# mlrun/mlrun

Measured on NVIDIA H100. Metric: events/sec, higher is better.
Workload: dtype f32 in / f64 accumulate

## Files before the change

### mlrun_b200/csrc/b2s_rowthread.cuh

```cuda
#pragma once
#include <cuda.h>
#include <type_traits>

#include "b2s_device.cuh"
#include "b2s_hash.cuh"

namespace b2s {

constexpr int kRTMaxCatCols = 16;
constexpr int kRTCatsInline = 4;
constexpr int kRTMaxCats = 256;

template <int NCH, int NS>
struct RTParams {
  const char* rows;
  int64_t row_stride;
  int64_t n_rows;
  float* out;
  int32_t* status;
  int32_t n_in, out_cols, n_models, vote_kind, out_is_int, fast_epilogue, tile_rows, pitch, stages, vec_ok;
  int32_t n_cat_cols, n_cat;
  int32_t one_sync;
  int32_t use_bulk;
  float* peers[8];
  int64_t peer_off;
  int32_t n_peers;
  MergeSig sig;
  const double* wcat;
  const double* vote_w_g;
  const ModelDesc* models;
  const int32_t* classes;
  double w[NCH * 4][NS];
  float fill[NCH * 4];
  float lim[NCH * 4];
  double bias[NS];
  double vote_w[NS];
  int32_t cat_col[kRTMaxCatCols];
  int32_t cat_off[kRTMaxCatCols];
  int32_t cat_sw[kRTMaxCatCols];
  int32_t cat_base[kRTMaxCatCols];
  int32_t cat_cnt[kRTMaxCatCols];
  float cat_fill[kRTMaxCatCols];
  float cat_inl[kRTMaxCatCols][kRTCatsInline];
  int32_t cat_first[kRTMaxCatCols];
  int32_t cat_dense[kRTMaxCatCols];
  float cat_val[kRTMaxCats];
  struct CatFast {
    int32_t off_b;
    int32_t sw_b;
    int32_t first;
    int32_t cnt;
    int32_t woff_b;
    float fill;
    int32_t pad[2];
  };
  CatFast catf[kRTMaxCatCols];
  int32_t cats_fast;
  int32_t zero_woff_b;
  int32_t dead_tail;
  int32_t pad_fast;
  const long long* g_keys;
  const TableSlot* g_slots;
  uint64_t g_mask;
  const float* g_values;
  long long g_missing_row;
};

struct RowPadded {
  const float* xr;
  __device__ __forceinline__ float4 chunk(int ch) const { return *reinterpret_cast<const float4*>(xr + ch * 4); }
  __device__ __forceinline__ float at2(int off, int) const { return xr[off]; }
  __device__ __forceinline__ float at_b(int off_b, int) const { return *reinterpret_cast<const float*>(reinterpret_cast<const char*>(xr) + off_b); }
};
struct RowSwizzled {
  const float* box0;
  int box_words;
  int r7s;
  __device__ __forceinline__ float4 chunk(int ch) const {
    return *reinterpret_cast<const float4*>(box0 + (ch >> 3) * box_words + (((ch & 7) << 2) ^ r7s));
  }
  __device__ __forceinline__ float at2(int off, int sw) const { return box0[off + (sw ^ r7s)]; }
  __device__ __forceinline__ float at_b(int off_b, int sw_b) const {
    return *reinterpret_cast<const float*>(reinterpret_cast<const char*>(box0) + off_b + (sw_b ^ (r7s << 2)));
  }
};

template <int NCH, int NS, int CH0, int CH1, typename Row>
__device__ __forceinline__ void rt_slice(const RTParams<NCH, NS>& p, const Row (&xr)[1], double (&acc)[1][NS]) {
  constexpr int RPT = 1;
  constexpr int BATCH = 4;
#pragma unroll
  for (int b = CH0; b < CH1; b += BATCH) {
    double xd[RPT][BATCH * 4];
#pragma unroll
    for (int cb = 0; cb < BATCH; ++cb) {
      const int ch = b + cb;
      if (ch < CH1) {
#pragma unroll
        for (int i = 0; i < RPT; ++i) {
          const float4 v = xr[i].chunk(ch);
          const float xs[4] = {v.x, v.y, v.z, v.w};
#pragma unroll
          for (int u = 0; u < 4; ++u) {
            const int c = ch * 4 + u;
            float x = xs[u];
            x = !(fabsf(x) <= p.lim[c]) ? p.fill[c] : x;
            xd[i][cb * 4 + u] = (double)x;
          }
        }
      }
    }
#pragma unroll
    for (int cb = 0; cb < BATCH; ++cb) {
      const int ch = b + cb;
      if (ch < CH1) {
#pragma unroll
        for (int u = 0; u < 4; ++u) {
          const int c = ch * 4 + u;
#pragma unroll
          for (int k = 0; k < NS; ++k)
#pragma unroll
            for (int i = 0; i < RPT; ++i) acc[i][k] = fma(p.w[c][k], xd[i][cb * 4 + u], acc[i][k]);
        }
      }
    }
  }
}

template <int NCH, int NS>
__device__ __noinline__ int rt_cat_search(const RTParams<NCH, NS>& p, int cc, float x) {
  const int b0 = p.cat_base[cc], cnt = p.cat_cnt[cc];
  int j = p.n_cat;
  if (cnt <= kRTCatsInline) {
#pragma unroll
    for (int qq = kRTCatsInline - 1; qq >= 0; --qq) j = (x == p.cat_inl[cc][qq]) ? b0 + qq : j;
  } else {
    for (int qq = cnt - 1; qq >= 0; --qq) j = (x == p.cat_val[b0 + qq]) ? b0 + qq : j;
  }
  return j;
}

template <int NCH, int NS, int Q0, int TPR, typename Row>
__device__ __forceinline__ void rt_cats(const RTParams<NCH, NS>& p, const Row (&xr)[1], const double* __restrict__ s_wcat,
                                        double (&acc)[1][NS]) {
  constexpr int RPT = 1;
  constexpr int ITERS = (kRTMaxCatCols - Q0 + TPR - 1) / TPR;
  if (p.cats_fast) {
    const char* wb = reinterpret_cast<const char*>(s_wcat);
#pragma unroll
    for (int it = 0; it < ITERS; ++it) {
      const int cc = Q0 + it * TPR;
      if (cc >= p.n_cat_cols) break;
      const typename RTParams<NCH, NS>::CatFast cf = p.catf[cc];
#pragma unroll
      for (int i = 0; i < RPT; ++i) {
        float x = xr[i].at_b(cf.off_b, cf.sw_b);
        x = (x != x) ? cf.fill : x;
        const int v = __float2int_rz(x);
        const unsigned jj = (unsigned)(v - cf.first);
        const bool miss = ((float)v != x) | (jj >= (unsigned)cf.cnt);
        const int a = miss ? p.zero_woff_b : cf.woff_b + (int)jj * (NS * 8);
        if constexpr (NS % 2 == 0) {
#pragma unroll
          for (int k = 0; k < NS; k += 2) {
            const double2 w2 = *reinterpret_cast<const double2*>(wb + a + k * 8);
            acc[i][k] += w2.x;
            acc[i][k + 1] += w2.y;
          }
        } else {
          const double* wc = reinterpret_cast<const double*>(wb + a);
#pragma unroll
          for (int k = 0; k < NS; ++k) acc[i][k] += wc[k];
        }
      }
    }
    return;
  }
#pragma unroll
  for (int it = 0; it < ITERS; ++it) {
    const int cc = Q0 + it * TPR;
    if (cc >= p.n_cat_cols) break;
#pragma unroll
    for (int i = 0; i < RPT; ++i) {
      float x = xr[i].at2(p.cat_off[cc], p.cat_sw[cc]);
      x = (x != x) ? p.cat_fill[cc] : x;
      int j;
      if (p.cat_dense[cc]) {
        const int v = __float2int_rz(x);
        const unsigned jj = (unsigned)(v - p.cat_first[cc]);
        j = ((float)v == x && jj < (unsigned)p.cat_cnt[cc]) ? p.cat_base[cc] + (int)jj : p.n_cat;
      } else {
        j = rt_cat_search(p, cc, x);
      }
      const double* wc = s_wcat + (size_t)j * NS;
#pragma unroll
      for (int k = 0; k < NS; ++k) acc[i][k] += wc[k];
    }
  }
}

template <int NCH, int NS, int TPR, int LIVE, typename Row>
__device__ __forceinline__ void rt_row_slices(const RTParams<NCH, NS>& p, int q, const Row (&xr)[1], const double* __restrict__ s_wcat,
                                              double (&acc)[1][NS]) {
  static_assert(LIVE % TPR == 0, "live chunks must split evenly over the row's threads");
  constexpr int CPT = LIVE / TPR;
  if (TPR == 1 || q == 0) {
    rt_slice<NCH, NS, 0, CPT>(p, xr, acc);
    rt_cats<NCH, NS, 0, TPR>(p, xr, s_wcat, acc);
  } else if (q == 1) {
    rt_slice<NCH, NS, (TPR > 1 ? CPT : 0), (TPR > 1 ? 2 * CPT : 0)>(p, xr, acc);
    rt_cats<NCH, NS, (TPR > 1 ? 1 : 0), TPR>(p, xr, s_wcat, acc);
  } else if (q == 2) {
    rt_slice<NCH, NS, (TPR > 2 ? 2 * CPT : 0), (TPR > 2 ? 3 * CPT : 0)>(p, xr, acc);
    rt_cats<NCH, NS, (TPR > 2 ? 2 : 0), TPR>(p, xr, s_wcat, acc);
  } else {
    rt_slice<NCH, NS, (TPR > 3 ? 3 * CPT : 0), (TPR > 3 ? 4 * CPT : 0)>(p, xr, acc);
    rt_cats<NCH, NS, (TPR > 3 ? 3 : 0), TPR>(p, xr, s_wcat, acc);
  }
}

__device__ __forceinline__ void mbar_init(uint64_t* bar, int count) {
  asm volatile("mbarrier.init.shared::cta.b64 [%0], %1;" ::"r"((uint32_t)__cvta_generic_to_shared(bar)), "r"(count));
}
__device__ __forceinline__ void mbar_expect_tx(uint64_t* bar, uint32_t bytes) {
  asm volatile("mbarrier.arrive.expect_tx.shared::cta.b64 _, [%0], %1;" ::"r"((uint32_t)__cvta_generic_to_shared(bar)), "r"(bytes)
               : "memory");
}
__device__ __forceinline__ void mbar_wait(uint64_t* bar, uint32_t parity) {
  const uint32_t a = (uint32_t)__cvta_generic_to_shared(bar);
  asm volatile(
      "{\n"
      ".reg .pred p;\n"
      "WAIT_%=:\n"
      "mbarrier.try_wait.parity.shared::cta.b64 p, [%0], %1;\n"
      "@p bra DONE_%=;\n"
      "bra WAIT_%=;\n"
      "DONE_%=:\n"
      "}\n" ::"r"(a), "r"(parity)
      : "memory");
}
__device__ __forceinline__ void bulk_load(void* smem_dst, const void* gsrc, uint32_t bytes, uint64_t* bar) {
  asm volatile("cp.async.bulk.shared::cluster.global.mbarrier::complete_tx::bytes [%0], [%1], %2, [%3];" ::"r"(
                   (uint32_t)__cvta_generic_to_shared(smem_dst)),
               "l"(gsrc), "r"(bytes), "r"((uint32_t)__cvta_generic_to_shared(bar))
               : "memory");
}

__device__ __forceinline__ void tensor_load_2d(void* smem_dst, const CUtensorMap* tmap, int x, int y, uint64_t* bar) {
  asm volatile(
      "cp.async.bulk.tensor.2d.shared::cluster.global.tile.mbarrier::complete_tx::bytes [%0], [%1, {%2, %3}], [%4];" ::"r"(
          (uint32_t)__cvta_generic_to_shared(smem_dst)),
      "l"(reinterpret_cast<uint64_t>(tmap)), "r"(x), "r"(y), "r"((uint32_t)__cvta_generic_to_shared(bar))
      : "memory");
}

template <int NCH, int NS>
__device__ __noinline__ void rt_generic_epilogue(const RTParams<NCH, NS>& p, const double* sl, int64_t row, uint32_t st) {
  double pred[kMaxModels];
  for (int m = 0; m < p.n_models; ++m) {
    const ModelDesc md = p.models[m];
    pred[m] = apply_link(md, sl + md.score_off, p.classes);
  }
  KParams kp;
  kp.out = p.out;
  kp.out_cols = p.out_cols;
  kp.n_models = p.n_models;
  kp.vote_kind = p.vote_kind;
  kp.out_is_int = p.out_is_int;
  kp.vote_w = p.vote_w_g;
  kp.status = p.status;
  kp.n_peers = p.n_peers;
  kp.peer_off = p.peer_off;
  for (int g = 0; g < p.n_peers; ++g) kp.peers[g] = p.peers[g];
  vote_and_store(kp, pred, row, st);
}

template <int NCH, int NS, int TPR, int LM>
__global__ void __launch_bounds__(128 * TPR, TPR >= 4 ? 2 : (TPR == 2 ? 3 : 4))
    rowthread_kernel(const __grid_constant__ RTParams<NCH, NS> p, const __grid_constant__ CUtensorMap tmap) {
  constexpr int RPT = 1;
  static_assert(NCH % TPR == 0, "chunks must split evenly over the row's threads");
  constexpr int CPT = NCH / TPR;
  extern __shared__ __align__(16) unsigned char smem[];
  uint64_t* s_bar = reinterpret_cast<uint64_t*>(smem);
  double* s_wcat = reinterpret_cast<double*>(smem + 64);
  const size_t wcat_bytes = 64 + (((size_t)(p.n_cat + 1) * NS * 8 + 15) / 16) * 16;
  const bool one_sync = (LM == 2) && TPR > 1 && p.one_sync;
  constexpr size_t part_words = (size_t)(TPR - 1) * 128 * NS;
  double* s_part = reinterpret_cast<double*>(smem + wcat_bytes);
  float* s_tiles = reinterpret_cast<float*>(smem + wcat_bytes + (one_sync ? 2 : 1) * part_words * 8);
  if (LM == 2) {
    const uint32_t a = (uint32_t)__cvta_generic_to_shared(s_tiles);
    s_tiles += ((1024u - (a & 1023u)) & 1023u) >> 2;
  }

  const int tid = threadIdx.x;
  const int TR = p.tile_rows;
  const int S = p.stages;
  const int tile_words = (LM == 2) ? TR * NCH * 4 : TR * p.pitch;
  const int64_t n_tiles = (p.n_rows + TR - 1) / TR;
  const int TRT = TR / RPT;
  const int q = tid / TRT;
  const int r = tid - q * TRT;

  const int cprv = p.vec_ok ? (p.n_in >> 2) : p.n_in;
  const int r0 = tid / cprv, c0 = tid - r0 * cprv;
  const int dr = (int)blockDim.x / cprv, dc = (int)blockDim.x - dr * cprv;
  auto issue = [&](float* tile, int64_t row0) {
    int64_t left = p.n_rows - row0;
    const int rows = left < TR ? (left < 0 ? 0 : (int)left) : TR;
    const char* base = p.rows + row0 * p.row_stride;
    int rr = r0, cc = c0;
    if (p.vec_ok) {
      while (rr < rows) {
        cp_async16(tile + rr * p.pitch + cc * 4, base + (int64_t)rr * p.row_stride + cc * 16);
        rr += dr;
        cc += dc;
        if (cc >= cprv) {
          cc -= cprv;
          ++rr;
        }
      }
    } else {
      while (rr < rows) {
        cp_async4(tile + rr * p.pitch + cc, base + (int64_t)rr * p.row_stride + cc * 4);
        rr += dr;
        cc += dc;
        if (cc >= cprv) {
          cc -= cprv;
          ++rr;
        }
      }
    }
  };

  constexpr bool bulk = LM != 0;
  const uint32_t row_bytes = (uint32_t)p.n_in * 4u;
  uint32_t unknown_bits = 0;
  long long gk_cur = 0, gk_nxt = 0;
  longlong2 g_slot = make_longlong2(0, -1);
  uint64_t g_hash = 0;
  int64_t g_tile_nxt = 0;
  auto g_key = [&](int64_t tile) -> long long {
    const int64_t row = tile * TR + tid;
    return row < p.n_rows ? __ldg(p.g_keys + row) : 0;
  };
  auto g_probe_start = [&](long long key) {
    g_hash = mix64((uint64_t)key) & p.g_mask;
    g_slot = __ldg(reinterpret_cast<const longlong2*>(p.g_slots) + g_hash);
  };
  auto g_probe_finish = [&](long long key) -> long long {
    uint64_t h = g_hash;
    longlong2 sl = g_slot;
    for (;;) {
      if (sl.y < 0) return -1;
      if (sl.x == key) return sl.y;
      h = (h + 1) & p.g_mask;
      sl = __ldg(reinterpret_cast<const longlong2*>(p.g_slots) + h);
    }
  };
  if (LM == 1 && p.g_keys && tid < TR) {
    gk_cur = g_key(blockIdx.x);
    gk_nxt = g_key((int64_t)blockIdx.x + gridDim.x);
    g_probe_start(gk_cur);
    g_tile_nxt = (int64_t)blockIdx.x + 2 * (int64_t)gridDim.x;
  }
  auto issue_bulk = [&](int st, int64_t row0) {
    int64_t left = p.n_rows - row0;
    const int rows = left < TR ? (left < 0 ? 0 : (int)left) : TR;
    if (LM == 2) {
      if (tid == 0) {
        if (rows > 0) {
          mbar_expect_tx(&s_bar[st], (uint32_t)(NCH / 8) * (uint32_t)TR * 128u);
#pragma unroll
          for (int b = 0; b < NCH / 8; ++b)
            tensor_load_2d(s_tiles + st * tile_words + b * TR * 32, &tmap, b * 32, (int)row0, &s_bar[st]);
        } else {
          mbar_expect_tx(&s_bar[st], 0);
        }
      }
    } else {
      if (tid == 0) mbar_expect_tx(&s_bar[st], (uint32_t)rows * row_bytes);
      if (p.g_keys) {
        if (tid < TR) {
          const long long hit = g_probe_finish(gk_cur);
          if (tid < rows) {
            unknown_bits = (unknown_bits & ~(1u << st)) | ((hit < 0 ? 1u : 0u) << st);
            bulk_load(s_tiles + st * tile_words + tid * p.pitch,
                      reinterpret_cast<const char*>(p.g_values + (hit < 0 ? p.g_missing_row : hit) * p.n_in), row_bytes, &s_bar[st]);
          }
          gk_cur = gk_nxt;
          g_probe_start(gk_cur);
          gk_nxt = g_key(g_tile_nxt);
          g_tile_nxt += gridDim.x;
        }
      } else if (tid < rows) {
        bulk_load(s_tiles + st * tile_words + tid * p.pitch, p.rows + (row0 + tid) * p.row_stride, row_bytes, &s_bar[st]);
      }
    }
  };
  if (bulk) {
    if (tid == 0) {
      for (int s = 0; s < S; ++s) mbar_init(&s_bar[s], 1);
      asm volatile("fence.mbarrier_init.release.cluster;" ::: "memory");
    }
    __syncthreads();
  }
  for (int s = 0; s < (one_sync ? S : S - 1); ++s) {
    const int64_t t = (int64_t)blockIdx.x + (int64_t)s * gridDim.x;
    if (bulk) {
      issue_bulk(s, t * TR);
    } else {
      if (t < n_tiles) issue(s_tiles + s * tile_words, t * TR);
      cp_async_commit();
    }
  }
  uint32_t phase_bits = 0;
  for (int i = tid; i < p.n_cat * NS; i += blockDim.x) s_wcat[i] = p.wcat[i];
  for (int i = tid; i < NS; i += blockDim.x) s_wcat[p.n_cat * NS + i] = 0.0;
  if (one_sync) __syncthreads();

  int stage = 0;
  uint32_t iter = 0;
  for (int64_t t = blockIdx.x; t < n_tiles; t += gridDim.x) {
    if (bulk) {
      mbar_wait(&s_bar[stage], (phase_bits >> stage) & 1u);
      phase_bits ^= (1u << stage);
    } else if (S == 2) cp_async_wait<0>();
    else if (S == 3) cp_async_wait<1>();
    else cp_async_wait<2>();
    if (!one_sync) {
      __syncthreads();
      const int64_t tn = t + (int64_t)(S - 1) * gridDim.x;
      int sn = stage + S - 1;
      if (sn >= S) sn -= S;
      if (bulk) {
        issue_bulk(sn, tn * TR);
      } else {
        if (tn < n_tiles) issue(s_tiles + sn * tile_words, tn * TR);
        cp_async_commit();
      }
    }
    const float* tile = s_tiles + stage * tile_words;
    const int64_t row0 = t * TR;
    const int live_rows = (int)(p.n_rows - row0 < (int64_t)TR ? p.n_rows - row0 : (int64_t)TR);
    const bool any_live = r < live_rows;
    using Row = typename std::conditional<LM == 2, RowSwizzled, RowPadded>::type;
    Row xr[RPT];
#pragma unroll
    for (int i = 0; i < RPT; ++i) {
      const int ri = r + i * TRT;
      if constexpr (LM == 2) {
        xr[i].box0 = tile + ri * 32;
        xr[i].box_words = TR * 32;
        xr[i].r7s = (r & 7) << 2;
      } else {
        xr[i].xr = tile + ri * p.pitch;
      }
    }
    double acc[RPT][NS];
#pragma unroll
    for (int i = 0; i < RPT; ++i)
#pragma unroll
      for (int k = 0; k < NS; ++k) acc[i][k] = 0.0;
    if (any_live) {
      if constexpr (LM == 2 && RPT == 1 && NCH >= 8 && (TPR == 1 || TPR == 2)) {
        if (p.dead_tail >= 4) rt_row_slices<NCH, NS, TPR, NCH - 4>(p, q, xr, s_wcat, acc);
        else if (p.dead_tail >= 2) rt_row_slices<NCH, NS, TPR, NCH - 2>(p, q, xr, s_wcat, acc);
        else rt_row_slices<NCH, NS, TPR, NCH>(p, q, xr, s_wcat, acc);
      } else {
        rt_row_slices<NCH, NS, TPR, NCH>(p, q, xr, s_wcat, acc);
      }
    }
    if (TPR > 1) {
      double* s_part_cur = s_part + (one_sync ? (size_t)(iter & 1) * part_words : 0);
      if (q > 0) {
#pragma unroll
        for (int i = 0; i < RPT; ++i) {
          double* part = s_part_cur + ((size_t)(q - 1) * 128 + r + i * TRT) * NS;
#pragma unroll
          for (int k = 0; k < NS; ++k) part[k] = acc[i][k];
        }
      }
      __syncthreads();
      if (one_sync) issue_bulk(stage, (t + (int64_t)S * gridDim.x) * TR);
      if (q == 0) {
#pragma unroll
        for (int i = 0; i < RPT; ++i)
#pragma unroll
          for (int qq = 1; qq < TPR; ++qq) {
            const double* o = s_part_cur + ((size_t)(qq - 1) * 128 + r + i * TRT) * NS;
#pragma unroll
            for (int k = 0; k < NS; ++k) acc[i][k] += o[k];
          }
      }
    }
#pragma unroll
    for (int i = 0; i < RPT; ++i) {
      const int64_t row = row0 + (r + i * TRT);
      if (q == 0 && r + i * TRT < live_rows) {
        uint32_t st = 0;
#pragma unroll
        for (int k = 0; k < NS; ++k) {
          acc[i][k] += p.bias[k];
          st |= (fabs(acc[i][k]) <= 1.7976931348623157e308) ? 0u : 1u;
        }
        if (LM == 1) st |= ((unknown_bits >> stage) & 1u) << 2;
        if (p.fast_epilogue) {
          if (p.vote_kind == 1) {
            double s = 0.0;
#pragma unroll
            for (int k = 0; k < NS; ++k) s = __dadd_rn(s, __dmul_rn(acc[i][k], p.vote_w[k]));
            store_word(p, row, 0, __float_as_uint((float)s));
          } else {
#pragma unroll
            for (int k = 0; k < NS; ++k)
              if (k < p.n_models) store_word(p, row, k, __float_as_uint((float)acc[i][k]));
          }
          if (p.status) p.status[row] = (int32_t)st;
        } else {
          double sl[NS];
#pragma unroll
          for (int k = 0; k < NS; ++k) sl[k] = acc[i][k];
          rt_generic_epilogue(p, sl, row, st);
        }
      }
    }
    ++stage;
    ++iter;
    if (stage == S) stage = 0;
  }
  cp_async_wait<0>();
  merge_signal(p.sig);
}

}
```

### mlrun_b200/csrc/b2s_runtime.cu

```cuda
#include <cuda_runtime.h>

#include <exception>

#include <algorithm>
#include <atomic>
#include <chrono>
#include <cmath>
#include <condition_variable>
#include <cstdarg>
#include <cstdio>
#include <cstdlib>
#include <cstring>
#include <deque>
#include <limits>
#include <map>
#include <memory>
#include <mutex>
#include <string>
#include <thread>
#include <vector>

#include "../../include/b200serve.h"
#include "b2s_internal.h"
#include "b2s_device.cuh"
// ... 113 lines not shown

struct b2s_plan_s {
  int32_t n_in = 0;
  bool finalized = false;
  std::vector<float> fill;
  std::vector<std::vector<MapEntry>> maps;
  std::vector<int32_t> out_src, out_kind;
  std::vector<float> out_arg;
  std::vector<HostModel> models;
  int vote_kind = B2S_VOTE_NONE;
  std::vector<double> vote_w;
  int mode = MODE_STORE;
  int NS = 1;
  int out_cols = 0;
  int out_is_int = 0;
  KParams kp{};
  char* d_blob = nullptr;
  size_t blob_bytes = 0;
  int grid = 0, block = 0;
  int kernels_per_batch = 1;
  bool rt_ok = false;
  int rt_cat_cols = 0;
  int rt_NCH = 0, rt_NS = 0, rt_grid = 0, rt_smem = 0, rt_pitch = 0;
  std::vector<char> rt_blob;
  std::vector<void*> peers;
  int64_t peer_off = 0;
  struct b2s_comm_s* comm = nullptr;
  bool t2_ok = false;
  int t2_NS = 1, t2_grid = 0, t2_block = 512, t2_smem = 0;
  T2Params t2{};
  char* d_t2_blob = nullptr;
  struct TreeScratch {
    double* pred = nullptr;
    int32_t* row_bad = nullptr;
    uint32_t* xt = nullptr;
    int64_t rows = 0;
  };
  std::map<cudaStream_t, TreeScratch> t2_scratch;
  std::mutex scratch_mu;
  bool dense_ok = false;
  DenseParams dense{};
  int dense_smem = 0, dense_grid = 0;
  std::atomic<int32_t> last_kernel{B2S_KERNEL_NONE};
  bool t3_ok = false, t3_miss = false, t3_cat = false;
  bool any_cat = false;
  int t3_D = 0, t3_grid = 0, t3_block = 0, t3_smem = 0, t3_cols = 0, t3_parts = 0;
  T3Params t3{};
  T3Prep t3_prep{};
  int t3_prep_smem = 0;
  char* d_t3_blob = nullptr;
  const int32_t* d_t3_col_score = nullptr;
  const int32_t* d_t3_col_order = nullptr;
  const int32_t* d_t3_model_cols = nullptr;
  char* h_stage_in = nullptr;
  char* h_stage_out = nullptr;
  char* d_stage_in = nullptr;
  char* d_stage_out = nullptr;
  int32_t* d_stage_status = nullptr;
  int64_t stage_rows = 0;
  cudaEvent_t ev[4] = {nullptr, nullptr, nullptr, nullptr};
  std::vector<cudaEvent_t> chunk_ev;
  std::mutex host_mu;
  std::vector<Slot> slots;
  int open_slot = -1;
  uint64_t next_batch = 1;
  std::map<uint64_t, int> batch_slot;
  std::deque<int> sealed;
  std::mutex mu;
  std::condition_variable cv_work, cv_done, cv_free;
  std::thread dispatcher;
  bool stop = false;
  bool dispatch_busy = false;
  cudaStream_t ring_stream = nullptr;
  int64_t ring_cap = 0;
  std::atomic<int> spinners{0};
  int ring_cfg_slots = 0;
  int64_t ring_cfg_max_batch = 0;
  int ring_cfg_wait_us = -1;
  int wait_us() const { return ring_cfg_wait_us >= 0 ? ring_cfg_wait_us : G.max_wait_us; }
};

int b2s_int_plan_shape(b2s_plan_s* p, int* n_in, int* out_cols) {
  if (!p || !p->finalized) return fail(B2S_ERR_STATE, "plan not finalized");
  *n_in = p->n_in;
  *out_cols = p->out_cols;
  return B2S_OK;
}

static size_t align_up(size_t x, size_t a) { return (x + a - 1) / a * a; }

struct BlobBuilder {
  std::vector<char> data;
  template <typename T>
  size_t add(const std::vector<T>& v) {
    size_t off = align_up(data.size(), 16);
    data.resize(off + std::max<size_t>(v.size() * sizeof(T), 16));
    if (!v.empty()) memcpy(data.data() + off, v.data(), v.size() * sizeof(T));
    return off;
  }
};

template <int MODE, int NS>
static cudaError_t launch_rows(const KParams& kp, int grid, int block, cudaStream_t st) {
  static std::atomic<bool> attr_set{false};
  if (!attr_set) {
    cudaError_t e = cudaFuncSetAttribute(rows_kernel<MODE, NS>, cudaFuncAttributeMaxDynamicSharedMemorySize,
                                         (int)G.prop.sharedMemPerBlockOptin);
    if (e != cudaSuccess) return e;
    attr_set = true;
  }
  rows_kernel<MODE, NS><<<grid, block, kp.sm_total, st>>>(kp);
  return cudaGetLastError();
}

static cudaError_t launch_plan(b2s_plan_s* p, const KParams& kp, int grid, int block, cudaStream_t st) {
  G.launches.fetch_add(1, std::memory_order_relaxed);
#define B2S_CASE(M, N) \
  if (p->mode == M && p->NS == N) return launch_rows<M, N>(kp, grid, block, st);
  B2S_CASE(MODE_LINEAR, 1) B2S_CASE(MODE_LINEAR, 2) B2S_CASE(MODE_LINEAR, 4) B2S_CASE(MODE_LINEAR, 8)
  B2S_CASE(MODE_LINEAR, 16) B2S_CASE(MODE_LINEAR, 32)
  B2S_CASE(MODE_TREES, 1) B2S_CASE(MODE_TREES, 4) B2S_CASE(MODE_TREES, 8) B2S_CASE(MODE_TREES, 16)
  B2S_CASE(MODE_TREES, 32) B2S_CASE(MODE_STORE, 1)
#undef B2S_CASE
  return cudaErrorInvalidValue;
}

typedef CUresult (*EncodeTiledFn)(CUtensorMap*, CUtensorMapDataType, cuuint32_t, void*, const cuuint64_t*, const cuuint64_t*,
                                  const cuuint32_t*, const cuuint32_t*, CUtensorMapInterleave, CUtensorMapSwizzle,
                                  CUtensorMapL2promotion, CUtensorMapFloatOOBfill);
static EncodeTiledFn tensor_map_encoder() {
  static EncodeTiledFn fn = [] {
    void* sym = nullptr;
    cudaDriverEntryPointQueryResult q;
    if (cudaGetDriverEntryPoint("cuTensorMapEncodeTiled", &sym, cudaEnableDefault, &q) != cudaSuccess || q != cudaDriverEntryPointSuccess) {
      cudaGetLastError();
      sym = nullptr;
    }
    return reinterpret_cast<EncodeTiledFn>(sym);
  }();
  return fn;
}
static bool encode_rows_map(CUtensorMap* map, const void* rows, int64_t n_rows, int64_t stride, int n_in, int tile_rows) {
  EncodeTiledFn enc = tensor_map_encoder();
  if (!enc) return false;
  cuuint64_t gdim[2] = {(cuuint64_t)n_in, (cuuint64_t)n_rows};
  cuuint64_t gstride[1] = {(cuuint64_t)stride};
  cuuint32_t box[2] = {32u, (cuuint32_t)tile_rows};
  cuuint32_t estr[2] = {1u, 1u};
  return enc(map, CU_TENSOR_MAP_DATA_TYPE_FLOAT32, 2, const_cast<void*>(rows), gdim, gstride, box, estr,
             CU_TENSOR_MAP_INTERLEAVE_NONE, CU_TENSOR_MAP_SWIZZLE_128B, CU_TENSOR_MAP_L2_PROMOTION_L2_128B,
             CU_TENSOR_MAP_FLOAT_OOB_FILL_NONE) == CUDA_SUCCESS;
}

struct RTTables {
  int n_in, n_out_cols, n_models, vote_kind, out_is_int, fast_epilogue, NS;
  const std::vector<float>* fill;
  const std::vector<uint32_t>* flags;
  const std::vector<double>* wnum;
  const std::vector<double>* bias;
  const std::vector<double>* vote_w;
  const std::vector<int32_t>* cat_off;
  const std::vector<float>* cat_val;
  const double* d_wcat;
  const double* d_vote_w;
  const ModelDesc* d_models;
  const int32_t* d_classes;
};

constexpr int rt_tpr(int NCH) { return NCH >= 8 ? 2 : 1; }
constexpr int kRTTileRows = 128, kRTStages = 2;

template <int NCH, int NS>
static void rt_build(b2s_plan_s* p, const RTTables& t) {
  using P = RTParams<NCH, NS>;
  p->rt_blob.assign(sizeof(P), 0);
  P& r = *reinterpret_cast<P*>(p->rt_blob.data());
  r.n_in = t.n_in;
  r.out_cols = t.n_out_cols;
  r.n_models = t.n_models;
  r.vote_kind = t.vote_kind;
  r.out_is_int = t.out_is_int;
  r.fast_epilogue = t.fast_epilogue;
  r.wcat = t.d_wcat;
  r.vote_w_g = t.d_vote_w;
  r.models = t.d_models;
  r.classes = t.d_classes;
  for (int c = 0; c < NCH * 4; ++c) {
    r.fill[c] = 0.0f;
    r.lim[c] = -1.0f;
    for (int k = 0; k < NS; ++k) r.w[c][k] = 0.0;
  }
  for (int c = 0; c < t.n_in; ++c) {
    const bool input = ((*t.flags)[c] & COL_COPIED) != 0;
    r.fill[c] = input ? (*t.fill)[c] : 0.0f;
    r.lim[c] = input ? std::numeric_limits<float>::infinity() : -1.0f;
    for (int k = 0; k < NS; ++k) r.w[c][k] = (*t.wnum)[(size_t)c * NS + k];
  }
  for (int k = 0; k < NS; ++k) {
    r.bias[k] = k < (int)t.bias->size() ? (*t.bias)[k] : 0.0;
    r.vote_w[k] = k < (int)t.vote_w->size() ? (*t.vote_w)[k] : 0.0;
  }
  int ncc = 0;
  for (int c = 0; c < t.n_in; ++c)
    if ((*t.cat_off)[c + 1] > (*t.cat_off)[c]) {
      r.cat_col[ncc] = c;
      r.cat_base[ncc] = (*t.cat_off)[c];
      r.cat_cnt[ncc] = (*t.cat_off)[c + 1] - (*t.cat_off)[c];
      r.cat_fill[ncc] = (*t.fill)[c];
      for (int q = 0; q < kRTCatsInline; ++q)
        r.cat_inl[ncc][q] = q < r.cat_cnt[ncc] ? (*t.cat_val)[r.cat_base[ncc] + q] : std::numeric_limits<float>::quiet_NaN();
      {
        const float f0 = (*t.cat_val)[r.cat_base[ncc]];
        bool dense = f0 == std::floor(f0) && std::fabs(f0) < 8388608.0f;
        for (int q = 0; dense && q < r.cat_cnt[ncc]; ++q) dense = (*t.cat_val)[r.cat_base[ncc] + q] == f0 + (float)q;
        r.cat_dense[ncc] = dense ? 1 : 0;
        r.cat_first[ncc] = dense ? (int)f0 : 0;
      }
      ++ncc;
    }
  r.n_cat_cols = ncc;
  r.n_cat = (int)t.cat_val->size();
  r.cats_fast = 1;
  for (int cc = 0; cc < ncc; ++cc) {
    r.cats_fast = r.cats_fast && r.cat_dense[cc];
    r.catf[cc].first = r.cat_first[cc];
    r.catf[cc].cnt = r.cat_cnt[cc];
    r.catf[cc].woff_b = r.cat_base[cc] * NS * 8;
    r.catf[cc].fill = r.cat_fill[cc];
  }
  r.zero_woff_b = r.n_cat * NS * 8;
  {
    int last_live = -1;
    for (int c = 0; c < t.n_in; ++c)
      if (((*t.flags)[c] & COL_COPIED) != 0) last_live = c >> 2;
    r.dead_tail = std::max(0, NCH - 1 - last_live);
    if (last_live < 0) r.dead_tail = 0;
  }
  for (int i = 0; i < r.n_cat; ++i) r.cat_val[i] = (*t.cat_val)[i];
}

struct LaunchCtx {
  const KParams* k = nullptr;
  bool host_rows = false;
};

template <int NCH, int NS>
static cudaError_t rt_launch_t(b2s_plan_s* p, const void* rows, int64_t stride, int64_t n_rows, void* out, int32_t* status,
                               int vec_ok, cudaStream_t st, bool query, int* occ, const B2SGather* gather, const LaunchCtx* lc) {
  using P = RTParams<NCH, NS>;
  constexpr int TPR = rt_tpr(NCH);
  constexpr int LMT = NCH >= 8 ? 2 : 1;
  static std::atomic<bool> attr_set{false};
  if (!attr_set) {
    const int cap = (int)G.prop.sharedMemPerBlockOptin;
    cudaError_t e = cudaFuncSetAttribute(rowthread_kernel<NCH, NS, TPR, 0>, cudaFuncAttributeMaxDynamicSharedMemorySize, cap);
    if (e == cudaSuccess) e = cudaFuncSetAttribute(rowthread_kernel<NCH, NS, TPR, 1>, cudaFuncAttributeMaxDynamicSharedMemorySize, cap);
    if (e == cudaSuccess && NCH >= 8)
      e = cudaFuncSetAttribute(rowthread_kernel<NCH, NS, TPR, LMT>, cudaFuncAttributeMaxDynamicSharedMemorySize, cap);
    if (e != cudaSuccess) return e;
    attr_set = true;
  }
  const bool tmap_ok = NCH >= 8 && p->n_in == NCH * 4 && tensor_map_encoder() != nullptr;
  if (query) {
    if (tmap_ok)
      return cudaOccupancyMaxActiveBlocksPerMultiprocessor(occ, rowthread_kernel<NCH, NS, TPR, LMT>, kRTTileRows * TPR, p->rt_smem);
    return cudaOccupancyMaxActiveBlocksPerMultiprocessor(occ, rowthread_kernel<NCH, NS, TPR, 0>, kRTTileRows * TPR, p->rt_smem);
  }
  P r = *reinterpret_cast<const P*>(p->rt_blob.data());
  r.rows = (const char*)rows;
  r.row_stride = stride;
  r.n_rows = n_rows;
  r.out = (float*)out;
  r.status = status;
  r.vec_ok = vec_ok;
  const KParams* lk = lc ? lc->k : nullptr;
  r.n_peers = lk ? lk->n_peers : (int)p->peers.size();
  r.peer_off = lk ? lk->peer_off : p->peer_off;
  for (int g = 0; g < r.n_peers; ++g) r.peers[g] = lk ? lk->peers[g] : (float*)p->peers[g];
  r.sig = lk ? lk->sig : MergeSig{};
  r.pitch = p->rt_pitch;
  r.stages = kRTStages;
  int mode = vec_ok ? 2 : 0;
  if (lc && lc->host_rows) mode = 0;
  if (mode == 2 && !tmap_ok) mode = 1;
  if (gather) {
    mode = 1;
    r.g_keys = gather->d_keys;
    r.g_slots = reinterpret_cast<const TableSlot*>(gather->d_slots);
    r.g_mask = gather->mask;
    r.g_values = gather->d_values;
    r.g_missing_row = gather->missing_row;
    if (gather->any_impute)
      for (int c = 0; c < p->n_in; ++c) {
        const float f = gather->h_impute[c];
        if (f == f && r.lim[c] == std::numeric_limits<float>::infinity()) {
          r.lim[c] = std::numeric_limits<float>::max();
          r.fill[c] = f;
        }
      }
  }
  int tr = kRTTileRows;
  while (tr > 32 && (n_rows + tr - 1) / tr < (int64_t)G.prop.multiProcessorCount) tr /= 2;
  alignas(64) CUtensorMap tmap;
  memset(&tmap, 0, sizeof(tmap));
  if (mode == 2 && !encode_rows_map(&tmap, rows, n_rows, stride, p->n_in, tr)) mode = 1;
  p->last_kernel.store(mode == 2 ? B2S_KERNEL_ROWTHREAD_TMA
                       : mode == 1 ? B2S_KERNEL_ROWTHREAD_BULK
                       : (lc && lc->host_rows) ? B2S_KERNEL_ROWTHREAD_HOST : B2S_KERNEL_ROWTHREAD_LDGSTS,
                       std::memory_order_relaxed);
  r.tile_rows = tr;
  const int64_t tiles = (n_rows + tr - 1) / tr;
  const int grid = (int)std::max<int64_t>(1, std::min<int64_t>(p->rt_grid, tiles));
  r.use_bulk = mode;
  r.one_sync = NS >= 4 ? 1 : 0;
  for (int cc = 0; cc < r.n_cat_cols; ++cc) {
    const int col = r.cat_col[cc], ch = col >> 2;
    r.cat_off[cc] = mode == 2 ? (ch >> 3) * (tr * 32) + (col & 3) : col;
    r.cat_sw[cc] = mode == 2 ? (ch & 7) << 2 : 0;
    r.catf[cc].off_b = r.cat_off[cc] * 4;
    r.catf[cc].sw_b = r.cat_sw[cc] * 4;
  }
  if (mode == 2)
    rowthread_kernel<NCH, NS, TPR, LMT><<<grid, tr * TPR, p->rt_smem, st>>>(r, tmap);
  else if (mode == 1)
    rowthread_kernel<NCH, NS, TPR, 1><<<grid, tr * TPR, p->rt_smem, st>>>(r, tmap);
  else
    rowthread_kernel<NCH, NS, TPR, 0><<<grid, tr * TPR, p->rt_smem, st>>>(r, tmap);
  return cudaGetLastError();
}

#define RT_DISPATCH(FN, ...)                                                              \
  do {                                                                                    \
    const int nch_ = p->rt_NCH, ns_ = p->rt_NS;                                           \
    if (nch_ == 4 && ns_ == 1) return FN<4, 1>(__VA_ARGS__);                              \
    if (nch_ == 4 && ns_ == 2) return FN<4, 2>(__VA_ARGS__);                              \
    if (nch_ == 4 && ns_ == 4) return FN<4, 4>(__VA_ARGS__);                              \
    if (nch_ == 4 && ns_ == 8) return FN<4, 8>(__VA_ARGS__);                              \
    if (nch_ == 8 && ns_ == 1) return FN<8, 1>(__VA_ARGS__);                              \
    if (nch_ == 8 && ns_ == 2) return FN<8, 2>(__VA_ARGS__);                              \
    if (nch_ == 8 && ns_ == 4) return FN<8, 4>(__VA_ARGS__);                              \
    if (nch_ == 8 && ns_ == 8) return FN<8, 8>(__VA_ARGS__);                              \
    if (nch_ == 16 && ns_ == 1) return FN<16, 1>(__VA_ARGS__);                            \
    if (nch_ == 16 && ns_ == 2) return FN<16, 2>(__VA_ARGS__);                            \
    if (nch_ == 16 && ns_ == 4) return FN<16, 4>(__VA_ARGS__);                            \
    if (nch_ == 16 && ns_ == 8) return FN<16, 8>(__VA_ARGS__);                            \
    if (nch_ == 32 && ns_ == 1) return FN<32, 1>(__VA_ARGS__);                            \
    if (nch_ == 32 && ns_ == 2) return FN<32, 2>(__VA_ARGS__);                            \
    if (nch_ == 32 && ns_ == 4) return FN<32, 4>(__VA_ARGS__);                            \
    if (nch_ == 32 && ns_ == 8) return FN<32, 8>(__VA_ARGS__);                            \
  } while (0)

static cudaError_t rt_launch(b2s_plan_s* p, const void* rows, int64_t stride, int64_t n_rows, void* out, int32_t* status,
                             int vec_ok, cudaStream_t st, bool query = false, int* occ = nullptr, const B2SGather* gather = nullptr,
                             const LaunchCtx* lc = nullptr) {
  RT_DISPATCH(rt_launch_t, p, rows, stride, n_rows, out, status, vec_ok, st, query, occ, gather, lc);
  return cudaErrorInvalidValue;
}
static void rt_build_any(b2s_plan_s* p, const RTTables& t) {
  RT_DISPATCH(rt_build, p, t);
}

extern "C" int b2s_version(void) { return B2S_VERSION; }
extern "C" const char* b2s_last_error(void) { return g_err.c_str(); }

extern "C" int b2s_init(int device_ordinal, const char* cfg) {
  try {
    std::lock_guard<std::mutex> lk(G.mu);
    if (G.inited) return B2S_OK;
    int n = 0;
    cudaError_t e = cudaGetDeviceCount(&n);
    if (e != cudaSuccess || n == 0)
      return fail(B2S_ERR_NO_DEVICE, "no CUDA device (%s); this engine has no CPU fallback",
                  e == cudaSuccess ? "device count 0" : cudaGetErrorString(e));
    if (device_ordinal < 0 || device_ordinal >= n) return fail(B2S_ERR_INVALID, "device ordinal %d out of range", device_ordinal);
    CUDA_TRY(cudaSetDevice(device_ordinal));
    CUDA_TRY(cudaGetDeviceProperties(&G.prop, device_ordinal));
    CUDA_TRY(cudaStreamCreateWithFlags(&G.stream, cudaStreamNonBlocking));
    CUDA_TRY(cudaStreamCreateWithFlags(&G.copy_stream, cudaStreamNonBlocking));
    G.device = device_ordinal;
    std::string c = cfg ? cfg : "";
    G.ring_slots = (int)cfg_get(c, "ring_slots", 4);
    G.max_batch = cfg_get(c, "max_batch", 65536);
    G.max_wait_us = cfg_get(c, "max_wait_us", 0);
    if (G.ring_slots < 2) G.ring_slots = 2;
    G.inited = true;
    return B2S_OK;
  } catch (const std::exception& e) {
    return fail(B2S_ERR_INVALID, "%s: %s", __func__, e.what());
  }
}

extern "C" int b2s_shutdown(void) {
  try {
    std::lock_guard<std::mutex> lk(G.mu);
    if (!G.inited) return B2S_OK;
    cudaStreamDestroy(G.stream);
    cudaStreamDestroy(G.copy_stream);
    G.stream = G.copy_stream = nullptr;
    G.inited = false;
    return B2S_OK;
  } catch (const std::exception& e) {
    return fail(B2S_ERR_INVALID, "%s: %s", __func__, e.what());
  }
}

extern "C" int b2s_device_info(b2s_devinfo* out) {
  try {
    if (!G.inited) return fail(B2S_ERR_STATE, "b2s_init was not called");
    if (!out) return fail(B2S_ERR_INVALID, "null out");
    memset(out, 0, sizeof(*out));
    out->ordinal = G.device;
    out->sm_count = G.prop.multiProcessorCount;
    out->cc_major = G.prop.major;
    out->cc_minor = G.prop.minor;
    out->total_mem = (int64_t)G.prop.totalGlobalMem;
    out->l2_bytes = G.prop.l2CacheSize;
    out->smem_per_block_optin = (int64_t)G.prop.sharedMemPerBlockOptin;
    strncpy(out->name, G.prop.name, sizeof(out->name) - 1);
    return B2S_OK;
  } catch (const std::exception& e) {
    return fail(B2S_ERR_INVALID, "%s: %s", __func__, e.what());
  }
}

extern "C" int64_t b2s_launch_count(void) { return G.launches.load(); }

extern "C" int b2s_plan_create(int32_t n_in_cols, b2s_plan_t* out) {
  try {
    if (!out || n_in_cols <= 0 || n_in_cols > 65536) return fail(B2S_ERR_INVALID, "bad n_in_cols %d", n_in_cols);
    auto* p = new b2s_plan_s();
    p->n_in = n_in_cols;
    p->fill.assign(n_in_cols, std::numeric_limits<float>::quiet_NaN());
    p->maps.resize(n_in_cols);
    *out = p;
    return B2S_OK;
  } catch (const std::exception& e) {
    return fail(B2S_ERR_INVALID, "%s: %s", __func__, e.what());
  }
}

static int check_build(b2s_plan_t p) {
  if (!p) return fail(B2S_ERR_INVALID, "null plan");
  if (p->finalized) return fail(B2S_ERR_STATE, "plan already finalized");
  return B2S_OK;
}

extern "C" int b2s_plan_set_impute(b2s_plan_t p, const int32_t* cols, const float* fills, int32_t n) {
  try {
    if (int rc = check_build(p)) return rc;
    for (int i = 0; i < n; ++i) {
      if (cols[i] < 0 || cols[i] >= p->n_in) return fail(B2S_ERR_INVALID, "impute column %d out of range", cols[i]);
      p->fill[cols[i]] = fills[i];
    }
    return B2S_OK;
  } catch (const std::exception& e) {
    return fail(B2S_ERR_INVALID, "%s: %s", __func__, e.what());
  }
}

extern "C" int b2s_plan_add_value_map(b2s_plan_t p, int32_t col, const float* keys, const float* vals, int32_t n) {
  try {
    if (int rc = check_build(p)) return rc;
    if (col < 0 || col >= p->n_in) return fail(B2S_ERR_INVALID, "map column %d out of range", col);
    for (int i = 0; i < n; ++i) p->maps[col].push_back(MapEntry{keys[i], 0.f, vals[i], (i == 0 ? 256 : 0) | 0});
    return B2S_OK;
  } catch (const std::exception& e) {
    return fail(B2S_ERR_INVALID, "%s: %s", __func__, e.what());
  }
}

extern "C" int b2s_plan_add_range_map(b2s_plan_t p, int32_t col, const float* lo, const float* hi, const float* vals, int32_t n) {
  try {
    if (int rc = check_build(p)) return rc;
    if (col < 0 || col >= p->n_in) return fail(B2S_ERR_INVALID, "map column %d out of range", col);
    for (int i = 0; i < n; ++i) p->maps[col].push_back(MapEntry{lo[i], hi[i], vals[i], (i == 0 ? 256 : 0) | 1});
    return B2S_OK;
  } catch (const std::exception& e) {
    return fail(B2S_ERR_INVALID, "%s: %s", __func__, e.what());
  }
}
// ... 2193 lines not shown
```

Before: 10.46 billion.

## Use 3D row-major TMA tiles, tensormap prefetch, and programmatic dependent launch

Replaces the per-32-column 2D TMA boxes with a single 3D tensor load per stage, so each row's chunks sit contiguously in shared memory with a per-row XOR swizzle, and updates the categorical offsets to match. It adds a tensormap prefetch and moves the shared-weight staging ahead of the main loop. It also launches through cudaLaunchKernelEx with programmatic stream serialization, using griddepcontrol wait and launch_dependents so that the next kernel's prologue can overlap this kernel's tail. The risks are swizzle-index mistakes and PDL ordering hazards if a dependent kernel reads outputs early.

```diff
diff --git a/mlrun_b200/csrc/b2s_rowthread.cuh b/mlrun_b200/csrc/b2s_rowthread.cuh
--- a/mlrun_b200/csrc/b2s_rowthread.cuh
+++ b/mlrun_b200/csrc/b2s_rowthread.cuh
@@ -73,15 +73,14 @@
   __device__ __forceinline__ float at_b(int off_b, int) const { return *reinterpret_cast<const float*>(reinterpret_cast<const char*>(xr) + off_b); }
 };
 struct RowSwizzled {
-  const float* box0;
-  int box_words;
+  const float* row;
   int r7s;
   __device__ __forceinline__ float4 chunk(int ch) const {
-    return *reinterpret_cast<const float4*>(box0 + (ch >> 3) * box_words + (((ch & 7) << 2) ^ r7s));
-  }
-  __device__ __forceinline__ float at2(int off, int sw) const { return box0[off + (sw ^ r7s)]; }
+    return *reinterpret_cast<const float4*>(row + (ch >> 3) * 32 + ((((ch & 7) ^ (ch >> 3)) << 2) ^ r7s));
+  }
+  __device__ __forceinline__ float at2(int off, int sw) const { return row[off + (sw ^ r7s)]; }
   __device__ __forceinline__ float at_b(int off_b, int sw_b) const {
-    return *reinterpret_cast<const float*>(reinterpret_cast<const char*>(box0) + off_b + (sw_b ^ (r7s << 2)));
+    return *reinterpret_cast<const float*>(reinterpret_cast<const char*>(row) + off_b + (sw_b ^ (r7s << 2)));
   }
 };
 
@@ -253,6 +252,16 @@
       "l"(reinterpret_cast<uint64_t>(tmap)), "r"(x), "r"(y), "r"((uint32_t)__cvta_generic_to_shared(bar))
       : "memory");
 }
+__device__ __forceinline__ void tensor_load_3d(void* smem_dst, const CUtensorMap* tmap, int x, int y, int z, uint64_t* bar) {
+  asm volatile(
+      "cp.async.bulk.tensor.3d.shared::cluster.global.tile.mbarrier::complete_tx::bytes [%0], [%1, {%2, %3, %4}], [%5];" ::"r"(
+          (uint32_t)__cvta_generic_to_shared(smem_dst)),
+      "l"(reinterpret_cast<uint64_t>(tmap)), "r"(x), "r"(y), "r"(z), "r"((uint32_t)__cvta_generic_to_shared(bar))
+      : "memory");
+}
+
+__device__ __forceinline__ void grid_dependency_wait() { asm volatile("griddepcontrol.wait;" ::: "memory"); }
+__device__ __forceinline__ void grid_launch_dependents() { asm volatile("griddepcontrol.launch_dependents;" ::: "memory"); }
 
 template <int NCH, int NS>
 __device__ __noinline__ void rt_generic_epilogue(const RTParams<NCH, NS>& p, const double* sl, int64_t row, uint32_t st) {
@@ -359,22 +368,14 @@
       sl = __ldg(reinterpret_cast<const longlong2*>(p.g_slots) + h);
     }
   };
-  if (LM == 1 && p.g_keys && tid < TR) {
-    gk_cur = g_key(blockIdx.x);
-    gk_nxt = g_key((int64_t)blockIdx.x + gridDim.x);
-    g_probe_start(gk_cur);
-    g_tile_nxt = (int64_t)blockIdx.x + 2 * (int64_t)gridDim.x;
-  }
   auto issue_bulk = [&](int st, int64_t row0) {
     int64_t left = p.n_rows - row0;
     const int rows = left < TR ? (left < 0 ? 0 : (int)left) : TR;
     if (LM == 2) {
       if (tid == 0) {
         if (rows > 0) {
-          mbar_expect_tx(&s_bar[st], (uint32_t)(NCH / 8) * (uint32_t)TR * 128u);
-#pragma unroll
-          for (int b = 0; b < NCH / 8; ++b)
-            tensor_load_2d(s_tiles + st * tile_words + b * TR * 32, &tmap, b * 32, (int)row0, &s_bar[st]);
+          mbar_expect_tx(&s_bar[st], (uint32_t)TR * (uint32_t)NCH * 16u);
+          tensor_load_3d(s_tiles + st * tile_words, &tmap, 0, 0, (int)row0, &s_bar[st]);
         } else {
           mbar_expect_tx(&s_bar[st], 0);
         }
@@ -399,12 +400,20 @@
       }
     }
   };
-  if (bulk) {
-    if (tid == 0) {
-      for (int s = 0; s < S; ++s) mbar_init(&s_bar[s], 1);
-      asm volatile("fence.mbarrier_init.release.cluster;" ::: "memory");
-    }
-    __syncthreads();
+  if (bulk && tid == 0) {
+    for (int s = 0; s < S; ++s) mbar_init(&s_bar[s], 1);
+    asm volatile("fence.mbarrier_init.release.cluster;" ::: "memory");
+    if (LM == 2) asm volatile("prefetch.tensormap [%0];" ::"l"(reinterpret_cast<uint64_t>(&tmap)) : "memory");
+  }
+  for (int i = tid; i < p.n_cat * NS; i += blockDim.x) s_wcat[i] = p.wcat[i];
+  for (int i = tid; i < NS; i += blockDim.x) s_wcat[p.n_cat * NS + i] = 0.0;
+  if (bulk) __syncthreads();
+  grid_dependency_wait();
+  if (LM == 1 && p.g_keys && tid < TR) {
+    gk_cur = g_key(blockIdx.x);
+    gk_nxt = g_key((int64_t)blockIdx.x + gridDim.x);
+    g_probe_start(gk_cur);
+    g_tile_nxt = (int64_t)blockIdx.x + 2 * (int64_t)gridDim.x;
   }
   for (int s = 0; s < (one_sync ? S : S - 1); ++s) {
     const int64_t t = (int64_t)blockIdx.x + (int64_t)s * gridDim.x;
@@ -416,9 +425,6 @@
     }
   }
   uint32_t phase_bits = 0;
-  for (int i = tid; i < p.n_cat * NS; i += blockDim.x) s_wcat[i] = p.wcat[i];
-  for (int i = tid; i < NS; i += blockDim.x) s_wcat[p.n_cat * NS + i] = 0.0;
-  if (one_sync) __syncthreads();
 
   int stage = 0;
   uint32_t iter = 0;
@@ -451,9 +457,8 @@
     for (int i = 0; i < RPT; ++i) {
       const int ri = r + i * TRT;
       if constexpr (LM == 2) {
-        xr[i].box0 = tile + ri * 32;
-        xr[i].box_words = TR * 32;
-        xr[i].r7s = (r & 7) << 2;
+        xr[i].row = tile + ri * (NCH * 4);
+        xr[i].r7s = ((ri * (NCH / 8)) & 7) << 2;
       } else {
         xr[i].xr = tile + ri * p.pitch;
       }
@@ -526,6 +531,7 @@
         }
       }
     }
+    if (t + (int64_t)S * gridDim.x >= n_tiles) grid_launch_dependents();
     ++stage;
     ++iter;
     if (stage == S) stage = 0;
diff --git a/mlrun_b200/csrc/b2s_runtime.cu b/mlrun_b200/csrc/b2s_runtime.cu
--- a/mlrun_b200/csrc/b2s_runtime.cu
+++ b/mlrun_b200/csrc/b2s_runtime.cu
@@ -289,6 +289,18 @@
              CU_TENSOR_MAP_FLOAT_OOB_FILL_NONE) == CUDA_SUCCESS;
 }
 
+static bool encode_row_tiles_map(CUtensorMap* map, const void* rows, int64_t n_rows, int64_t stride, int NCH, int tile_rows) {
+  EncodeTiledFn enc = tensor_map_encoder();
+  if (!enc) return false;
+  cuuint64_t gdim[3] = {32u, (cuuint64_t)(NCH / 8), (cuuint64_t)n_rows};
+  cuuint64_t gstride[2] = {128u, (cuuint64_t)stride};
+  cuuint32_t box[3] = {32u, (cuuint32_t)(NCH / 8), (cuuint32_t)tile_rows};
+  cuuint32_t estr[3] = {1u, 1u, 1u};
+  return enc(map, CU_TENSOR_MAP_DATA_TYPE_FLOAT32, 3, const_cast<void*>(rows), gdim, gstride, box, estr,
+             CU_TENSOR_MAP_INTERLEAVE_NONE, CU_TENSOR_MAP_SWIZZLE_128B, CU_TENSOR_MAP_L2_PROMOTION_L2_128B,
+             CU_TENSOR_MAP_FLOAT_OOB_FILL_NONE) == CUDA_SUCCESS;
+}
+
 struct RTTables {
   int n_in, n_out_cols, n_models, vote_kind, out_is_int, fast_epilogue, NS;
   const std::vector<float>* fill;
@@ -440,7 +452,7 @@
   while (tr > 32 && (n_rows + tr - 1) / tr < (int64_t)G.prop.multiProcessorCount) tr /= 2;
   alignas(64) CUtensorMap tmap;
   memset(&tmap, 0, sizeof(tmap));
-  if (mode == 2 && !encode_rows_map(&tmap, rows, n_rows, stride, p->n_in, tr)) mode = 1;
+  if (mode == 2 && !encode_row_tiles_map(&tmap, rows, n_rows, stride, NCH, tr)) mode = 1;
   p->last_kernel.store(mode == 2 ? B2S_KERNEL_ROWTHREAD_TMA
                        : mode == 1 ? B2S_KERNEL_ROWTHREAD_BULK
                        : (lc && lc->host_rows) ? B2S_KERNEL_ROWTHREAD_HOST : B2S_KERNEL_ROWTHREAD_LDGSTS,
@@ -452,17 +464,27 @@
   r.one_sync = NS >= 4 ? 1 : 0;
   for (int cc = 0; cc < r.n_cat_cols; ++cc) {
     const int col = r.cat_col[cc], ch = col >> 2;
-    r.cat_off[cc] = mode == 2 ? (ch >> 3) * (tr * 32) + (col & 3) : col;
-    r.cat_sw[cc] = mode == 2 ? (ch & 7) << 2 : 0;
+    r.cat_off[cc] = mode == 2 ? (ch >> 3) * 32 + (col & 3) : col;
+    r.cat_sw[cc] = mode == 2 ? ((ch & 7) ^ (ch >> 3)) << 2 : 0;
     r.catf[cc].off_b = r.cat_off[cc] * 4;
     r.catf[cc].sw_b = r.cat_sw[cc] * 4;
   }
+  cudaLaunchAttribute attr[1];
+  attr[0].id = cudaLaunchAttributeProgrammaticStreamSerialization;
+  attr[0].val.programmaticStreamSerializationAllowed = 1;
+  cudaLaunchConfig_t cfg = {};
+  cfg.gridDim = dim3(grid);
+  cfg.blockDim = dim3(tr * TPR);
+  cfg.dynamicSmemBytes = p->rt_smem;
+  cfg.stream = st;
+  cfg.attrs = attr;
+  cfg.numAttrs = 1;
   if (mode == 2)
-    rowthread_kernel<NCH, NS, TPR, LMT><<<grid, tr * TPR, p->rt_smem, st>>>(r, tmap);
+    cudaLaunchKernelEx(&cfg, rowthread_kernel<NCH, NS, TPR, LMT>, r, tmap);
   else if (mode == 1)
-    rowthread_kernel<NCH, NS, TPR, 1><<<grid, tr * TPR, p->rt_smem, st>>>(r, tmap);
+    cudaLaunchKernelEx(&cfg, rowthread_kernel<NCH, NS, TPR, 1>, r, tmap);
   else
-    rowthread_kernel<NCH, NS, TPR, 0><<<grid, tr * TPR, p->rt_smem, st>>>(r, tmap);
+    cudaLaunchKernelEx(&cfg, rowthread_kernel<NCH, NS, TPR, 0>, r, tmap);
   return cudaGetLastError();
 }
 
```

New measurement: 10.53 billion, median of 6. No clear change (+0.7%).

## Enable programmatic dependent launch and tensormap/L2 prefetch for TMA rowthread kernel

Applied to the files above, without the earlier changes.

For the TMA row-loading path, the kernel now launches with programmatic stream serialization. The prologue (tensormap prefetch, L2 prefetch of the first tiles, loading categorical weights into shared memory) runs before griddepcontrol.wait, so it can overlap the tail of the previous kernel. Each block signals launch_dependents once it has issued its last tile load, letting the next launch start early. This targets launch gaps between back-to-back kernels. It relies on prior kernels' writes not being needed before the wait, and it is limited to launches with no peers or signals.

```diff
diff --git a/mlrun_b200/csrc/b2s_rowthread.cuh b/mlrun_b200/csrc/b2s_rowthread.cuh
--- a/mlrun_b200/csrc/b2s_rowthread.cuh
+++ b/mlrun_b200/csrc/b2s_rowthread.cuh
@@ -403,8 +403,24 @@
     if (tid == 0) {
       for (int s = 0; s < S; ++s) mbar_init(&s_bar[s], 1);
       asm volatile("fence.mbarrier_init.release.cluster;" ::: "memory");
+      if (LM == 2) asm volatile("prefetch.tensormap [%0];" ::"l"(reinterpret_cast<uint64_t>(&tmap)) : "memory");
     }
     __syncthreads();
+  }
+  if (LM == 2) {
+    for (int i = tid; i < p.n_cat * NS; i += blockDim.x) s_wcat[i] = p.wcat[i];
+    for (int i = tid; i < NS; i += blockDim.x) s_wcat[p.n_cat * NS + i] = 0.0;
+    if (tid == 0)
+      for (int s = 0; s < (one_sync ? S : S - 1); ++s) {
+        const int64_t t = (int64_t)blockIdx.x + (int64_t)s * gridDim.x;
+        if (t * TR < p.n_rows)
+#pragma unroll
+          for (int b = 0; b < NCH / 8; ++b)
+            asm volatile("cp.async.bulk.prefetch.tensor.2d.L2.global.tile [%0, {%1, %2}];" ::"l"(reinterpret_cast<uint64_t>(&tmap)),
+                         "r"(b * 32), "r"((int)(t * TR))
+                         : "memory");
+      }
+    asm volatile("griddepcontrol.wait;" ::: "memory");
   }
   for (int s = 0; s < (one_sync ? S : S - 1); ++s) {
     const int64_t t = (int64_t)blockIdx.x + (int64_t)s * gridDim.x;
@@ -416,8 +432,10 @@
     }
   }
   uint32_t phase_bits = 0;
-  for (int i = tid; i < p.n_cat * NS; i += blockDim.x) s_wcat[i] = p.wcat[i];
-  for (int i = tid; i < NS; i += blockDim.x) s_wcat[p.n_cat * NS + i] = 0.0;
+  if (LM != 2) {
+    for (int i = tid; i < p.n_cat * NS; i += blockDim.x) s_wcat[i] = p.wcat[i];
+    for (int i = tid; i < NS; i += blockDim.x) s_wcat[p.n_cat * NS + i] = 0.0;
+  }
   if (one_sync) __syncthreads();
 
   int stage = 0;
@@ -436,6 +454,7 @@
       if (sn >= S) sn -= S;
       if (bulk) {
         issue_bulk(sn, tn * TR);
+        if (LM == 2 && tn + gridDim.x >= n_tiles) asm volatile("griddepcontrol.launch_dependents;" ::: "memory");
       } else {
         if (tn < n_tiles) issue(s_tiles + sn * tile_words, tn * TR);
         cp_async_commit();
@@ -483,7 +502,11 @@
         }
       }
       __syncthreads();
-      if (one_sync) issue_bulk(stage, (t + (int64_t)S * gridDim.x) * TR);
+      if (one_sync) {
+        const int64_t tn = t + (int64_t)S * gridDim.x;
+        issue_bulk(stage, tn * TR);
+        if (tn + gridDim.x >= n_tiles) asm volatile("griddepcontrol.launch_dependents;" ::: "memory");
+      }
       if (q == 0) {
 #pragma unroll
         for (int i = 0; i < RPT; ++i)
diff --git a/mlrun_b200/csrc/b2s_runtime.cu b/mlrun_b200/csrc/b2s_runtime.cu
--- a/mlrun_b200/csrc/b2s_runtime.cu
+++ b/mlrun_b200/csrc/b2s_runtime.cu
@@ -457,7 +457,19 @@
     r.catf[cc].off_b = r.cat_off[cc] * 4;
     r.catf[cc].sw_b = r.cat_sw[cc] * 4;
   }
-  if (mode == 2)
+  if (mode == 2 && r.n_peers == 0 && r.sig.n == 0) {
+    cudaLaunchConfig_t cfg = {};
+    cudaLaunchAttribute attr[1];
+    attr[0].id = cudaLaunchAttributeProgrammaticStreamSerialization;
+    attr[0].val.programmaticStreamSerializationAllowed = 1;
+    cfg.gridDim = dim3(grid);
+    cfg.blockDim = dim3(tr * TPR);
+    cfg.dynamicSmemBytes = p->rt_smem;
+    cfg.stream = st;
+    cfg.attrs = attr;
+    cfg.numAttrs = 1;
+    return cudaLaunchKernelEx(&cfg, rowthread_kernel<NCH, NS, TPR, LMT>, r, tmap);
+  } else if (mode == 2)
     rowthread_kernel<NCH, NS, TPR, LMT><<<grid, tr * TPR, p->rt_smem, st>>>(r, tmap);
   else if (mode == 1)
     rowthread_kernel<NCH, NS, TPR, 1><<<grid, tr * TPR, p->rt_smem, st>>>(r, tmap);
```

After: 10.46 billion before, 10.71 billion after (median of 6 runs). 2.3% higher.
